# spygaurad/Transformer-CNN-Hybrid-Network-for-Video-Processing

Hardware: AMD Instinct MI355X
Metric: clips/sec fwd+bwd, [B=8,T=16,3,224,224] d=512, 1/2/4/8 MI355X (higher is better)
Workload: dtype bf16; 1 GPU; config 2: clips [8,16,3,224,224] per GPU, CNN 32-64-128-256 + 2-layer transformer d=512 h=8 hid=2048, 8 classes; global_batch=8, frames=16, step=zero_grad+fwd+cross_entropy+bwd+grad_allreduce+adamw, launch=1 replayed hipGraph per step (graph.GraphedTrainStep), optimizer=HybridAdamW (hyb_adamw_step, one launch), parallelism=dp1, train_mode=BatchNorm batch stats, attention dropout 0.1 (reference semantics)

## Files before the change

transformer_cnn_hybrid_network_for_video_processing_amd/csrc/conv_v2.hip:

```cpp
#include <stdlib.h>
#include <type_traits>
#include "hyb_common.h"

namespace {

typedef __attribute__((address_space(3))) void lds_void_t;

template <int N> __device__ __forceinline__ void wait_vmcnt() { asm volatile("s_waitcnt vmcnt(%0)" ::"n"(N) : "memory"); }

__device__ __forceinline__ void dma16(__amdgpu_buffer_rsrc_t rsrc, unsigned voff, unsigned soff, bf16* lds_dst_wave_base) {
    __builtin_amdgcn_raw_ptr_buffer_load_lds(rsrc, (lds_void_t*)lds_dst_wave_base, 16, voff, soff, 0, 0);
}
constexpr unsigned V2_OOB = 0xfffffff0u;
constexpr unsigned V2_RECORDS = 0x80000000u;

template <int S> using step_c = std::integral_constant<int, S>;

template <int NT, int CB, int PGR, int PGC, int R>
struct V2Geom {
    static constexpr int PG = PGR * PGC, MT = 7;
    static constexpr int NW = CB * PG;
    static constexpr int TH = 4 * PGR, TW = 28 * PGC, HH = TH + 2, HW_ = TW + 2, HP = HH * HW_;
    static constexpr int NHW = (HP * 4 + 63) / 64;
    static constexpr int HT = (NHW + NW - 1) / NW;
    static constexpr int HBUF = NHW * 512;
    static constexpr int CBW = CB * NT * 16;
    static constexpr int WSLOT = CBW * 32;
    static constexpr int NWW = CBW / 16;
    static constexpr int WI = NWW >= NW ? NWW / NW : 1;
    static constexpr int NHS = 10 - R;
    static constexpr int STAT_FLOATS = NW * 2 * NT * 16;
    static constexpr size_t LDS_BYTES = (size_t)(2 * HBUF + R * WSLOT) * 2 + STAT_FLOATS * 4;
    static_assert(NW == 8 || NW == 4, "four or eight waves");
    static_assert(LDS_BYTES <= (NW == 8 ? 160 : 80) * 1024, "160 KiB of LDS per CU");
    static_assert(HW_ % 4 == 2, "halo swizzle assumes halo width = 2 mod 4");
    static_assert(R >= 3 && R <= 6, "ring depth");
    static constexpr int hi(int s) { s = ((s % 9) + 9) % 9; return s < NHS ? (HT + NHS - 1 - s) / NHS : 0; }
    static constexpr int hstart(int s) { int a = 0; for (int j = 0; j < s; ++j) a += hi(j); return a; }
    static constexpr int wait_n(int s) {
        int n = hi(s - R + 3);
        for (int j = s - R + 4; j <= s; ++j) n += WI + hi(j);
        return n;
    }
};

template <int NT, int CB, int PGR, int PGC, int R, bool STATS>
__global__ __launch_bounds__(CB * PGR * PGC * 64, CB * PGR * PGC == 4 ? 2 : 1) void conv3x3_v2_kernel(const bf16* __restrict__ x, const bf16* __restrict__ wp,
                                                            bf16* __restrict__ y, float* __restrict__ stats,
                                                            int N, int H, int W, int Cip, int Cop,
                                                            int tilesX, int tilesY, int numTiles, int stat_rows, int xpix, long long xblk) {
    using G = V2Geom<NT, CB, PGR, PGC, R>;
    constexpr int MT = G::MT, TH = G::TH, TW = G::TW, HW_ = G::HW_, HP = G::HP, HT = G::HT, NHW = G::NHW;
    constexpr int CBW = G::CBW, WSLOT = G::WSLOT, NWW = G::NWW, WI = G::WI, PG = G::PG, NW = G::NW, NTHR = NW * 64;
    extern __shared__ __attribute__((aligned(16))) unsigned char smem_raw[];
    bf16* const hbuf = reinterpret_cast<bf16*>(smem_raw);
    bf16* const wring = hbuf + 2 * G::HBUF;
    float* const wgstat = reinterpret_cast<float*>(wring + R * WSLOT);

    const int tid = threadIdx.x;
    const int lane = tid & 63;
    const int wave = __builtin_amdgcn_readfirstlane(tid >> 6);
    const int cb = wave % CB, pg = wave / CB;
    const int prow = pg / PGC, pstrip = pg % PGC;
    const int p = lane & 15, q = lane >> 4, py = p >> 2, px = p & 3;
    const int co_wg = blockIdx.y * CBW;
    const int co_base = co_wg + cb * (NT * 16);
    const int nCblk = Cip / 32;
    const long long wrow = (long long)9 * Cip;

    if (STATS) {
        for (int i = tid; i < G::STAT_FLOATS; i += NTHR) wgstat[i] = 0.f;
    }

    constexpr bool HOFF_REG = true;
    unsigned hoff[HOFF_REG ? HT : 1];
    int hyx[HT];
#pragma unroll
    for (int k = 0; k < HT; ++k) {
        int wi = k * NW + wave;
        if (wi > NHW - 1) wi = NHW - 1;
        const int u = wi * 64 + lane, hp = u >> 2, sp = u & 3;
        const int hy = hp / HW_, hx = hp - hy * HW_;
        const int s = sp ^ ((hy & 1) << 1);
        if (HOFF_REG) hoff[k] = (unsigned)(((hy * W + hx) * xpix + s * 8) * 2);
        hyx[k] = hp < HP ? ((hy << 20) | (hx << 4) | s) : (0x7ff << 20);
    }
    unsigned woff[WI];
    int wdst[WI];
#pragma unroll
    for (int i = 0; i < WI; ++i) {
        const int wi = (i * NW + wave) % NWW;
        const int u = wi * 64 + lane, row = u >> 2, sp = u & 3;
        const int f = (4 - ((row >> 3) & 3)) & 3;
        woff[i] = (unsigned)(((long long)row * wrow + ((sp ^ f) << 3)) * 2);
        wdst[i] = wi * 512;
    }
    const __amdgpu_buffer_rsrc_t wrsrc = hyb_rsrc((wp + (long long)co_wg * wrow), V2_RECORDS);
    const int aoff0 = (cb * (NT * 16) + (p >> 2) * 8 + (p & 3)) * 32 + ((q ^ ((4 - (p >> 2)) & 3)) << 3);
    auto aoff = [&](int t) { return aoff0 + ((t >> 1) * 32 + (t & 1) * 4) * 32; };
    const int lane_el = ((prow * 4 + py) * HW_ + pstrip * 28 + px) * 32;

    struct Blk { int n, ty0, tx0, cblk; };
    auto decode = [&](int tile, int cblk) {
        Blk b;
        b.n = tile / (tilesX * tilesY);
        const int trem = tile - b.n * (tilesX * tilesY);
        b.ty0 = (trem / tilesX) * TH;
        b.tx0 = (trem % tilesX) * TW;
        b.cblk = cblk;
        return b;
    };
    auto halo_rsrc = [&](const Blk& b) {
        const long long base = ((long long)(b.n * H + b.ty0 - 1) * W + (b.tx0 - 1)) * xpix + b.cblk * xblk;
        return hyb_rsrc((x + base), V2_RECORDS);
    };
    auto halo_piece = [&](const Blk& b, __amdgpu_buffer_rsrc_t rs, bf16* hb, int k) {
        const int hy = hyx[k] >> 20, hx = (hyx[k] >> 4) & 0xffff;
        const int gy = b.ty0 - 1 + hy, gx = b.tx0 - 1 + hx;
        const bool valid = ((unsigned)gy < (unsigned)H) && ((unsigned)gx < (unsigned)W);
        const unsigned off = HOFF_REG ? hoff[HOFF_REG ? k : 0] : (unsigned)(((hy * W + hx) * xpix + (hyx[k] & 15) * 8) * 2);
        int wi = k * NW + wave;
        if (wi > NHW - 1) wi = NHW - 1;
        dma16(rs, valid ? off : V2_OOB, 0, hb + wi * 512);
    };
    auto weight_pieces = [&](int cblk, int tap, int slot) {
        const unsigned so = (unsigned)((cblk * 9 + tap) * 64);
#pragma unroll
        for (int i = 0; i < WI; ++i) dma16(wrsrc, woff[i], so, wring + slot * WSLOT + wdst[i]);
    };
    auto bptr_of = [&](const bf16* hb, int tap) {
        const int kh = tap / 3, kw = tap % 3;
        const int sw = ((py + kh) & 1) << 1;
        return hb + lane_el + (kh * HW_ + kw) * 32 + ((q ^ sw) << 3);
    };

    const int tchunk = (numTiles + (int)gridDim.x - 1) / (int)gridDim.x;
    int tile = blockIdx.x * tchunk;
    const int tile_end = tile + tchunk < numTiles ? tile + tchunk : numTiles;
    Blk cur = decode(tile, 0);
    int hsel = 0, slot_cur = 0;
    bool after_store = false;
    constexpr int NS = MT * ((NT + 1) / 2);

    {
        const __amdgpu_buffer_rsrc_t rs0 = halo_rsrc(cur);
#pragma unroll
        for (int k = 0; k < HT; ++k) halo_piece(cur, rs0, hbuf, k);
    }
#pragma unroll
    for (int s = 0; s < R - 1; ++s) weight_pieces(0, s, s);
    wait_vmcnt<0>();
    __builtin_amdgcn_s_barrier();

    Frag<bf16> a_cur[NT], bfr[MT];
#pragma unroll
    for (int t = 0; t < NT; ++t) frag_load(a_cur[t], wring + aoff(t));
    {
        const bf16* bp = bptr_of(hbuf, 0);
#pragma unroll
        for (int m = 0; m < MT; ++m) frag_load(bfr[m], bp + m * 128);
    }

    f32x4 acc[MT][NT];
#pragma unroll
    for (int m = 0; m < MT; ++m)
#pragma unroll
        for (int t = 0; t < NT; ++t) acc[m][t] = f32x4{0.f, 0.f, 0.f, 0.f};

    while (true) {
        const bool last_cblk = cur.cblk + 1 >= nCblk;
        const int ntile = last_cblk ? (tile + 1 < tile_end ? tile + 1 : tile) : tile;
        const Blk nxt = decode(ntile, last_cblk ? 0 : cur.cblk + 1);
        bf16* const hb_cur = hbuf + hsel * G::HBUF;
        bf16* const hb_nxt = hbuf + (hsel ^ 1) * G::HBUF;
        const __amdgpu_buffer_rsrc_t nrs = halo_rsrc(nxt);

        auto step = [&](auto S_) __attribute__((always_inline)) {
            constexpr int S = decltype(S_)::value;
            {
                constexpr int FT = (S + R - 1) % 9;
                const int fc = (S + R - 1 >= 9) ? nxt.cblk : cur.cblk;
                int slot_fill = slot_cur - 1;
                if (slot_fill < 0) slot_fill += R;
                weight_pieces(fc, FT, slot_fill);
#pragma unroll
                for (int k = 0; k < G::hi(S); ++k) halo_piece(nxt, nrs, hb_nxt, G::hstart(S) + k);
            }
            int slot_next = slot_cur + 1;
            if (slot_next >= R) slot_next -= R;
            Frag<bf16> a_nxt[NT];
            {
                const bf16* as = wring + slot_next * WSLOT;
#pragma unroll
                for (int t = 0; t < NT; ++t) frag_load(a_nxt[t], as + aoff(t));
            }
            const bf16* bp = bptr_of(S == 8 ? hb_nxt : hb_cur, (S + 1) % 9);
#pragma unroll
            for (int m = 0; m < MT; ++m) {
#pragma unroll
                for (int t = 0; t < NT; ++t) acc[m][t] = mma32(a_cur[t], bfr[m], acc[m][t]);
                frag_load(bfr[m], bp + m * 128);
            }
#pragma unroll
            for (int m = 0; m < MT; ++m) {
                __builtin_amdgcn_sched_group_barrier(0x008, NT, 0);
                if (m < NT) __builtin_amdgcn_sched_group_barrier(0x100, 2, 0);
                else __builtin_amdgcn_sched_group_barrier(0x100, 1, 0);
            }
#pragma unroll
            for (int t = 0; t < NT; ++t) a_cur[t] = a_nxt[t];
            slot_cur = slot_next;
            if constexpr (S < R - 3) {
                if (after_store) wait_vmcnt<G::wait_n(S) + NS>(); else wait_vmcnt<G::wait_n(S)>();
            } else {
                wait_vmcnt<G::wait_n(S)>();
            }
            __builtin_amdgcn_s_barrier();
        };
        step(step_c<0>{}); step(step_c<1>{}); step(step_c<2>{}); step(step_c<3>{}); step(step_c<4>{});
        step(step_c<5>{}); step(step_c<6>{}); step(step_c<7>{}); step(step_c<8>{});

        if (last_cblk) {
            const int n = cur.n, ty0 = cur.ty0, tx0 = cur.tx0;
            const bool full = (ty0 + TH <= H) && (tx0 + TW <= W);
            float s1[NT][4], s2[NT][4];
            if (STATS) {
#pragma unroll
                for (int t = 0; t < NT; ++t)
#pragma unroll
                    for (int r = 0; r < 4; ++r) { s1[t][r] = 0.f; s2[t][r] = 0.f; }
            }
            const int gy = ty0 + prow * 4 + py;
            auto emit = [&](auto FULL_) __attribute__((always_inline)) {
                constexpr bool FULL = decltype(FULL_)::value;
#pragma unroll
                for (int m = 0; m < MT; ++m) {
                    const int gx = tx0 + pstrip * 28 + m * 4 + px;
                    const bool valid = FULL || ((gy < H) && (gx < W));
                    if (valid) {
                        bf16* dst = y + ((long long)(n * H + gy) * W + gx) * Cop + co_base + q * 8;
#pragma unroll
                        for (int h = 0; h < (NT + 1) / 2; ++h) {
                            Vec8<bf16> v;
#pragma unroll
                            for (int j = 0; j < 8; ++j) v.set(j, acc[m][NT == 1 ? 0 : h * 2 + (j >> 2)][j & 3]);
                            v.store(dst + h * 32);
                        }
                        if (STATS) {
#pragma unroll
                            for (int t = 0; t < NT; ++t)
#pragma unroll
                                for (int r = 0; r < 4; ++r) {
                                    const float v = acc[m][t][r];
                                    s1[t][r] += v;
                                    s2[t][r] = fmaf(v, v, s2[t][r]);
                                }
                        }
                    }
#pragma unroll
                    for (int t = 0; t < NT; ++t) acc[m][t] = f32x4{0.f, 0.f, 0.f, 0.f};
                }
            };
            if (full) {
                emit(std::true_type{});
                after_store = true;
            } else {
                emit(std::false_type{});
                wait_vmcnt<0>();
                after_store = false;
            }
            if (STATS) {
#pragma unroll
                for (int t = 0; t < NT; ++t)
#pragma unroll
                    for (int r = 0; r < 4; ++r) {
                        const float a = row16_sum(s1[t][r]), b = row16_sum(s2[t][r]);
                        if (p == 0) {
                            const int cl = (t >> 1) * 32 + q * 8 + (t & 1) * 4 + r;
                            wgstat[(wave * 2 + 0) * (NT * 16) + cl] += a;
                            wgstat[(wave * 2 + 1) * (NT * 16) + cl] += b;
                        }
                    }
            }
            if (tile + 1 >= tile_end) break;
            ++tile;
        }
        else after_store = false;
        cur = nxt;
        hsel ^= 1;
    }

    wait_vmcnt<0>();
    if (STATS) {
        __syncthreads();
        for (int i = tid; i < 2 * CBW; i += NTHR) {
            const int which = i / CBW, cl = i % CBW;
            const int cbi = cl / (NT * 16), c16 = cl % (NT * 16);
            float a = 0.f;
#pragma unroll
            for (int g = 0; g < PG; ++g) a += wgstat[((g * CB + cbi) * 2 + which) * (NT * 16) + c16];
            stats[((long long)blockIdx.x * 2 + which) * Cop + co_wg + cl] = a;
            for (int rrow = blockIdx.x + gridDim.x; rrow < stat_rows; rrow += gridDim.x) stats[((long long)rrow * 2 + which) * Cop + co_wg + cl] = 0.f;
        }
    }
}

template <int CB, int PGR, int PGC, bool STATS>
__global__ __launch_bounds__(CB * PGR * PGC * 64, 2) void conv3x3_k32_kernel(const bf16* __restrict__ x, const bf16* __restrict__ wp, bf16* __restrict__ y,
                                                                            float* __restrict__ stats, int N, int H, int W, int Cip, int Cop, int tilesX,
                                                                            int tilesY, int numTiles, int stat_rows, int xpix, long long xblk) {
    constexpr int NT = 2, HBN = 3;
    using G = V2Geom<NT, CB, PGR, PGC, 3>;
    constexpr int MT = G::MT, TH = G::TH, TW = G::TW, HW_ = G::HW_, HP = G::HP, HT = G::HT, NHW = G::NHW, CBW = G::CBW, PG = G::PG, NW = G::NW,
                  NTHR = NW * 64;
    static_assert(NW == 4, "two four-wave workgroups per CU");
    extern __shared__ __attribute__((aligned(16))) unsigned char smem_raw[];
    bf16* const hbuf = reinterpret_cast<bf16*>(smem_raw);
    float* const wgstat = reinterpret_cast<float*>(hbuf + HBN * G::HBUF);
    const int tid = threadIdx.x, lane = tid & 63;
    const int wave = __builtin_amdgcn_readfirstlane(tid >> 6);
    const int cb = wave % CB, pg = wave / CB;
    const int prow = pg / PGC, pstrip = pg % PGC;
    const int p = lane & 15, q = lane >> 4, py = p >> 2, px = p & 3;
    const int co_wg = blockIdx.y * CBW;
    const int co_base = co_wg + cb * (NT * 16);
    const long long wrow = (long long)9 * Cip;
    (void)xblk;

    Frag<bf16> aw[9][NT];
#pragma unroll
    for (int t = 0; t < NT; ++t) {
        const bf16* row = wp + (long long)(co_base + (t >> 1) * 32 + (p >> 2) * 8 + (t & 1) * 4 + (p & 3)) * wrow + 8 * q;
#pragma unroll
        for (int tap = 0; tap < 9; ++tap) frag_load(aw[tap][t], row + tap * 32);
    }
    unsigned hoff[HT];
    int hyx[HT];
#pragma unroll
    for (int k = 0; k < HT; ++k) {
        int wi = k * NW + wave;
        if (wi > NHW - 1) wi = NHW - 1;
        const int u = wi * 64 + lane, hp = u >> 2, sp = u & 3;
        const int hy = hp / HW_, hx = hp - hy * HW_;
        const int s = sp ^ ((hy & 1) << 1);
        hoff[k] = (unsigned)(((hy * W + hx) * xpix + s * 8) * 2);
        hyx[k] = hp < HP ? ((hy << 20) | (hx << 4) | s) : (0x7ff << 20);
    }
    const int lane_el = ((prow * 4 + py) * HW_ + pstrip * 28 + px) * 32;
    struct Tl { int n, ty0, tx0; };
    auto decode = [&](int tile) {
        Tl b;
        b.n = tile / (tilesX * tilesY);
        const int trem = tile - b.n * (tilesX * tilesY);
        b.ty0 = (trem / tilesX) * TH;
        b.tx0 = (trem % tilesX) * TW;
        return b;
    };
    auto halo_dma = [&](const Tl& b, bf16* hb) {
        const long long base = ((long long)(b.n * H + b.ty0 - 1) * W + (b.tx0 - 1)) * xpix;
        const __amdgpu_buffer_rsrc_t rs = hyb_rsrc((x + base), V2_RECORDS);
#pragma unroll
        for (int k = 0; k < HT; ++k) {
            const int hy = hyx[k] >> 20, hx = (hyx[k] >> 4) & 0xffff;
            const int gy = b.ty0 - 1 + hy, gx = b.tx0 - 1 + hx;
            const bool valid = ((unsigned)gy < (unsigned)H) && ((unsigned)gx < (unsigned)W);
            int wi = k * NW + wave;
            if (wi > NHW - 1) wi = NHW - 1;
            dma16(rs, valid ? hoff[k] : V2_OOB, 0, hb + wi * 512);
        }
    };
    auto bptr_of = [&](const bf16* hb, int tap) {
        const int kh = tap / 3, kw = tap % 3;
        const int sw = ((py + kh) & 1) << 1;
        return hb + lane_el + (kh * HW_ + kw) * 32 + ((q ^ sw) << 3);
    };

    const int tchunk = (numTiles + (int)gridDim.x - 1) / (int)gridDim.x;
    const int tile0 = blockIdx.x * tchunk;
    const int tile_end = tile0 + tchunk < numTiles ? tile0 + tchunk : numTiles;
    const int ntiles = tile_end - tile0;
    auto tl = [&](int i) { return decode(tile0 + (i < ntiles ? i : ntiles - 1)); };
    constexpr int NS = MT * ((NT + 1) / 2);

    halo_dma(tl(0), hbuf);
    halo_dma(tl(1), hbuf + G::HBUF);
    wait_vmcnt<0>();
    __builtin_amdgcn_s_barrier();

    Frag<bf16> bfr[MT];
    {
        const bf16* bp = bptr_of(hbuf, 0);
#pragma unroll
        for (int m = 0; m < MT; ++m) frag_load(bfr[m], bp + m * 128);
    }
    f32x4 acc[MT][NT];
#pragma unroll
    for (int m = 0; m < MT; ++m)
#pragma unroll
        for (int t = 0; t < NT; ++t) acc[m][t] = f32x4{0.f, 0.f, 0.f, 0.f};
    float s1[NT][4], s2[NT][4];
#pragma unroll
    for (int t = 0; t < NT; ++t)
#pragma unroll
        for (int r = 0; r < 4; ++r) { s1[t][r] = 0.f; s2[t][r] = 0.f; }

    int hsel = 0;
    bool prev_full = false;
    for (int it = 0; it < ntiles; ++it) {
        const Tl cur = tl(it);
        const int h1 = hsel + 1 >= HBN ? 0 : hsel + 1, h2 = h1 + 1 >= HBN ? 0 : h1 + 1;
        const bf16* hb_cur = hbuf + hsel * G::HBUF;
        const bf16* hb_nxt = hbuf + h1 * G::HBUF;
        halo_dma(tl(it + 2), hbuf + h2 * G::HBUF);
#pragma unroll
        for (int tap = 0; tap < 9; ++tap) {
            const bf16* bp = bptr_of(tap == 8 ? hb_nxt : hb_cur, (tap + 1) % 9);
#pragma unroll
            for (int m = 0; m < MT; ++m) {
#pragma unroll
                for (int t = 0; t < NT; ++t) acc[m][t] = mma32(aw[tap][t], bfr[m], acc[m][t]);
                frag_load(bfr[m], bp + m * 128);
            }
#pragma unroll
            for (int m = 0; m < MT; ++m) {
                __builtin_amdgcn_sched_group_barrier(0x008, NT, 0);
                __builtin_amdgcn_sched_group_barrier(0x100, 1, 0);
            }
        }
        const int n = cur.n, ty0 = cur.ty0, tx0 = cur.tx0;
        const bool full = (ty0 + TH <= H) && (tx0 + TW <= W);
        const int gy = ty0 + prow * 4 + py;
        auto emit = [&](auto FULL_) __attribute__((always_inline)) {
            constexpr bool FULL = decltype(FULL_)::value;
#pragma unroll
            for (int m = 0; m < MT; ++m) {
                const int gx = tx0 + pstrip * 28 + m * 4 + px;
                const bool valid = FULL || ((gy < H) && (gx < W));
                if (valid) {
                    bf16* dst = y + ((long long)(n * H + gy) * W + gx) * Cop + co_base + q * 8;
                    Vec8<bf16> v;
#pragma unroll
                    for (int j = 0; j < 8; ++j) v.set(j, acc[m][j >> 2][j & 3]);
                    v.store(dst);
                    if (STATS) {
#pragma unroll
                        for (int t = 0; t < NT; ++t)
#pragma unroll
                            for (int r = 0; r < 4; ++r) {
                                const float a = acc[m][t][r];
                                s1[t][r] += a;
                                s2[t][r] = fmaf(a, a, s2[t][r]);
                            }
                    }
                }
#pragma unroll
                for (int t = 0; t < NT; ++t) acc[m][t] = f32x4{0.f, 0.f, 0.f, 0.f};
            }
        };
        if (full) {
            emit(std::true_type{});
            if (prev_full) wait_vmcnt<HT + 2 * NS>(); else wait_vmcnt<HT + NS>();
        } else {
            emit(std::false_type{});
            wait_vmcnt<0>();
        }
        prev_full = full;
        __builtin_amdgcn_s_barrier();
        hsel = h1;
    }
    wait_vmcnt<0>();
    if (STATS) {
#pragma unroll
        for (int t = 0; t < NT; ++t)
#pragma unroll
            for (int r = 0; r < 4; ++r) {
                const float a = row16_sum(s1[t][r]), b = row16_sum(s2[t][r]);
                if (p == 0) {
                    const int cl = (t >> 1) * 32 + q * 8 + (t & 1) * 4 + r;
                    wgstat[(wave * 2 + 0) * (NT * 16) + cl] = a;
                    wgstat[(wave * 2 + 1) * (NT * 16) + cl] = b;
                }
            }
        __syncthreads();
        for (int i = tid; i < 2 * CBW; i += NTHR) {
            const int which = i / CBW, cl = i % CBW;
            const int cbi = cl / (NT * 16), c16 = cl % (NT * 16);
            float a = 0.f;
#pragma unroll
            for (int g = 0; g < PG; ++g) a += wgstat[((g * CB + cbi) * 2 + which) * (NT * 16) + c16];
            stats[((long long)blockIdx.x * 2 + which) * Cop + co_wg + cl] = a;
            for (int rrow = blockIdx.x + gridDim.x; rrow < stat_rows; rrow += gridDim.x) stats[((long long)rrow * 2 + which) * Cop + co_wg + cl] = 0.f;
        }
    }
}

template <int CB, int PGR, int PGC>
int launch_k32(const bf16* x, const bf16* wp, bf16* y, float* part, int N, int H, int W, int Cip, int Cop, int stat_rows, hipStream_t st, int xpix,
               long long xblk) {
    using G = V2Geom<2, CB, PGR, PGC, 3>;
    constexpr size_t LDS = (size_t)3 * G::HBUF * 2 + G::STAT_FLOATS * 4;
    static_assert(LDS <= 80 * 1024, "two workgroups per CU");
    const int tilesX = hyb_cdiv(W, G::TW), tilesY = hyb_cdiv(H, G::TH);
    const long long numTiles = (long long)N * tilesX * tilesY;
    int gx = (int)(numTiles < 512 ? numTiles : 512);
    if (part && gx > stat_rows) gx = stat_rows;
    if (gx < 1) gx = 1;
    gx = hyb_cdiv(numTiles, hyb_cdiv(numTiles, gx));
    const dim3 grid(gx, Cop / G::CBW);
    static HybAttrOnce once_stats, once_plain;
    if (int e = hyb_set_lds_attr(once_stats, (const void*)conv3x3_k32_kernel<CB, PGR, PGC, true>, (int)LDS)) return e;
    if (int e = hyb_set_lds_attr(once_plain, (const void*)conv3x3_k32_kernel<CB, PGR, PGC, false>, (int)LDS)) return e;
    if (part)
        hipLaunchKernelGGL((conv3x3_k32_kernel<CB, PGR, PGC, true>), grid, dim3(256), LDS, st, x, wp, y, part, N, H, W, Cip, Cop, tilesX, tilesY, (int)numTiles,
                           stat_rows, xpix, xblk);
    else
        hipLaunchKernelGGL((conv3x3_k32_kernel<CB, PGR, PGC, false>), grid, dim3(256), LDS, st, x, wp, y, (float*)nullptr, N, H, W, Cip, Cop, tilesX, tilesY,
                           (int)numTiles, 0, xpix, xblk);
    HYB_LAUNCH_CHECK();
    return 0;
}

template <int NT, int CB, int PGR, int PGC, int R>
int launch_v2(const bf16* x, const bf16* wp, bf16* y, float* part, int N, int H, int W, int Cip, int Cop, int stat_rows, hipStream_t st, int xpix,
              long long xblk) {
    using G = V2Geom<NT, CB, PGR, PGC, R>;
    const int tilesX = hyb_cdiv(W, G::TW), tilesY = hyb_cdiv(H, G::TH);
    const long long numTiles = (long long)N * tilesX * tilesY;
    constexpr int SLOTS = G::NW == 8 ? 256 : 512;
    int gx = (int)(numTiles < SLOTS ? numTiles : SLOTS);
    if (part && gx > stat_rows) gx = stat_rows;
    if (gx < 1) gx = 1;
    gx = hyb_cdiv(numTiles, hyb_cdiv(numTiles, gx));
    const dim3 grid(gx, Cop / G::CBW);
    static HybAttrOnce once_stats, once_plain;
    if (int e = hyb_set_lds_attr(once_stats, (const void*)conv3x3_v2_kernel<NT, CB, PGR, PGC, R, true>, (int)G::LDS_BYTES)) return e;
    if (int e = hyb_set_lds_attr(once_plain, (const void*)conv3x3_v2_kernel<NT, CB, PGR, PGC, R, false>, (int)G::LDS_BYTES)) return e;
    if (part)
        hipLaunchKernelGGL((conv3x3_v2_kernel<NT, CB, PGR, PGC, R, true>), grid, dim3(G::NW * 64), G::LDS_BYTES, st, x, wp, y, part, N, H, W, Cip, Cop,
                           tilesX, tilesY, (int)numTiles, stat_rows, xpix, xblk);
    else
        hipLaunchKernelGGL((conv3x3_v2_kernel<NT, CB, PGR, PGC, R, false>), grid, dim3(G::NW * 64), G::LDS_BYTES, st, x, wp, y, (float*)nullptr, N, H, W,
                           Cip, Cop, tilesX, tilesY, (int)numTiles, 0, xpix, xblk);
    HYB_LAUNCH_CHECK();
    return 0;
}

double v2_cost(int N, int H, int W, int TH, int TW, int gy) {
    const long long tiles = (long long)N * hyb_cdiv(W, TW) * hyb_cdiv(H, TH) * gy;
    const long long rounds = (tiles + 255) / 256;
    return (double)rounds * TH * TW;
}

}

int hyb_conv_v2_supported(int W, int Cip, int Cop) {
    return !(Cip % 32 != 0 || (long long)40 * W * Cip >= (1ll << 29) || (long long)256 * 9 * Cip >= (1ll << 29)) && Cop % 32 == 0;
}

int hyb_conv_v2(const void* x, const void* wp, void* y, float* part, int N, int H, int W, int Cip, int Cop, int stat_rows, hipStream_t st, long long xblk) {
    const int xpix = xblk ? 32 : Cip;
    if (!xblk) xblk = 32;
    if (Cip % 32 != 0 || (long long)40 * W * Cip >= (1ll << 29) || (long long)256 * 9 * Cip >= (1ll << 29)) return -100;
    const bf16* xb = (const bf16*)x; const bf16* wb = (const bf16*)wp; bf16* yb = (bf16*)y;
#define V2(NT_, CB_, PGR_, PGC_, R_) launch_v2<NT_, CB_, PGR_, PGC_, R_>(xb, wb, yb, part, N, H, W, Cip, Cop, stat_rows, st, xpix, xblk)
    static const int nw_env = getenv("HYB_V2_NW") ? atoi(getenv("HYB_V2_NW")) : 0;
    const int nw = nw_env ? nw_env : (Cop % 256 == 0 ? 8 : 4);
    static const int k32_env = getenv("HYB_CONV_K32") ? atoi(getenv("HYB_CONV_K32")) : 1;
    if (k32_env && nw == 4 && Cip == 32 && Cop % 64 == 0) {
        return v2_cost(N, H, W, 8, 28, Cop / 64) <= v2_cost(N, H, W, 4, 56, Cop / 64)
                   ? launch_k32<2, 2, 1>(xb, wb, yb, part, N, H, W, Cip, Cop, stat_rows, st, xpix, xblk)
                   : launch_k32<2, 1, 2>(xb, wb, yb, part, N, H, W, Cip, Cop, stat_rows, st, xpix, xblk);
    }
    if (nw == 4) {
        if (Cop % 256 == 0) return V2(4, 4, 1, 1, 3);
        if (Cop % 128 == 0) return v2_cost(N, H, W, 8, 28, Cop / 128) <= v2_cost(N, H, W, 4, 56, Cop / 128) ? V2(4, 2, 2, 1, 4) : V2(4, 2, 1, 2, 4);
        if (Cop % 64 == 0) return v2_cost(N, H, W, 8, 28, Cop / 64) <= v2_cost(N, H, W, 4, 56, Cop / 64) ? V2(2, 2, 2, 1, 4) : V2(2, 2, 1, 2, 4);
        if (Cop % 32 == 0) return V2(2, 1, 4, 1, 4);
        return -100;
    }
    if (Cop % 256 == 0) {
        return v2_cost(N, H, W, 8, 28, Cop / 256) <= v2_cost(N, H, W, 4, 56, Cop / 256) ? V2(4, 4, 2, 1, 6) : V2(4, 4, 1, 2, 6);
    }
    if (Cop % 128 == 0) {
        return v2_cost(N, H, W, 16, 28, Cop / 128) <= v2_cost(N, H, W, 8, 56, Cop / 128) ? V2(4, 2, 4, 1, 6) : V2(4, 2, 2, 2, 6);
    }
    if (Cop % 64 == 0) return V2(4, 1, 4, 2, 5);
    if (Cop % 32 == 0) return V2(2, 1, 4, 2, 6);
#undef V2
    return -100;
}
```

Baseline: 6085 clips/s.

## Add 8-wave single-workgroup conv3x3 v3 kernel with row-streamed weight ring

Adds a conv3x3 kernel that runs one 512-thread workgroup per CU over four pixel groups. Weights are streamed one kernel row at a time through a three-slot LDS ring, and input halos are double-buffered, so DMA for the next row or channel block overlaps the MFMA work of the current one. The dispatcher sends Cop==128, Cip>=256 convolutions (such as the 256->128 data-gradient conv) to this kernel when 16-row tiles cost less than 8-row tiles. It trades the two-workgroups-per-CU occupancy of v2 for larger tiles with more weight reuse, which risks weaker latency hiding.

```diff
diff --git a/transformer_cnn_hybrid_network_for_video_processing_amd/csrc/conv_v2.hip b/transformer_cnn_hybrid_network_for_video_processing_amd/csrc/conv_v2.hip
--- a/transformer_cnn_hybrid_network_for_video_processing_amd/csrc/conv_v2.hip
+++ b/transformer_cnn_hybrid_network_for_video_processing_amd/csrc/conv_v2.hip
@@ -305,6 +305,285 @@
     }
 }
 
+template <int NT, int CB, int PGR, int PGC>
+struct V3Geom : V2Geom<NT, CB, PGR, PGC, 3> {
+    using B = V2Geom<NT, CB, PGR, PGC, 3>;
+    static constexpr int R = 3;
+    static constexpr int RSLOT = 3 * B::WSLOT;
+    static constexpr int WPS = 3 * B::WI;
+    static constexpr size_t LDS_BYTES = (size_t)(2 * B::HBUF + R * RSLOT) * 2 + B::STAT_FLOATS * 4;
+    static_assert(B::NW == 8 && B::PG == 4, "one 8-wave workgroup per CU, four pixel groups");
+    static_assert(LDS_BYTES <= 160 * 1024, "160 KiB of LDS per CU");
+    static_assert(B::HH <= 18, "32-bit halo offsets: hyb_conv_v2_supported bounds 40 * W * Cip");
+    static constexpr int wait_n(int s) { return (s == 0 ? B::HT : 0) + WPS; }
+    static_assert(wait_n(0) + B::MT * ((NT + 1) / 2) <= 63, "vmcnt range");
+};
+
+template <int NT, int CB, int PGR, int PGC, bool STATS>
+__global__ __launch_bounds__(512, 1) void conv3x3_v3_kernel(const bf16* __restrict__ x, const bf16* __restrict__ wp, bf16* __restrict__ y,
+                                                            float* __restrict__ stats, int N, int H, int W, int Cip, int Cop, int tilesX, int tilesY,
+                                                            int numTiles, int stat_rows, int xpix, long long xblk) {
+    using G = V3Geom<NT, CB, PGR, PGC>;
+    constexpr int MT = G::MT, TH = G::TH, TW = G::TW, HW_ = G::HW_, HP = G::HP, HT = G::HT, NHW = G::NHW;
+    constexpr int CBW = G::CBW, WSLOT = G::WSLOT, RSLOT = G::RSLOT, NWW = G::NWW, WI = G::WI, PG = G::PG, NW = G::NW, R = G::R, NTHR = NW * 64;
+    extern __shared__ __attribute__((aligned(16))) unsigned char smem_raw[];
+    bf16* const hbuf = reinterpret_cast<bf16*>(smem_raw);
+    bf16* const wring = hbuf + 2 * G::HBUF;
+    float* const wgstat = reinterpret_cast<float*>(wring + R * RSLOT);
+
+    const int tid = threadIdx.x;
+    const int lane = tid & 63;
+    const int wave = __builtin_amdgcn_readfirstlane(tid >> 6);
+    const int cb = wave % CB, pg = wave / CB;
+    const int prow = pg / PGC, pstrip = pg % PGC;
+    const int p = lane & 15, q = lane >> 4, py = p >> 2, px = p & 3;
+    const int co_wg = blockIdx.y * CBW;
+    const int co_base = co_wg + cb * (NT * 16);
+    const int nCblk = Cip / 32;
+    const long long wrow = (long long)9 * Cip;
+
+    if (STATS) {
+        for (int i = tid; i < G::STAT_FLOATS; i += NTHR) wgstat[i] = 0.f;
+    }
+
+    unsigned hoff[HT];
+    int hyx[HT];
+#pragma unroll
+    for (int k = 0; k < HT; ++k) {
+        int wi = k * NW + wave;
+        if (wi > NHW - 1) wi = NHW - 1;
+        const int u = wi * 64 + lane, hp = u >> 2, sp = u & 3;
+        const int hy = hp / HW_, hx = hp - hy * HW_;
+        const int s = sp ^ ((hy & 1) << 1);
+        hoff[k] = (unsigned)(((hy * W + hx) * xpix + s * 8) * 2);
+        hyx[k] = hp < HP ? ((hy << 20) | (hx << 4) | s) : (0x7ff << 20);
+    }
+    unsigned woff[WI];
+    int wdst[WI];
+#pragma unroll
+    for (int i = 0; i < WI; ++i) {
+        const int wi = (i * NW + wave) % NWW;
+        const int u = wi * 64 + lane, row = u >> 2, sp = u & 3;
+        const int f = (4 - ((row >> 3) & 3)) & 3;
+        woff[i] = (unsigned)(((long long)row * wrow + ((sp ^ f) << 3)) * 2);
+        wdst[i] = wi * 512;
+    }
+    const __amdgpu_buffer_rsrc_t wrsrc = hyb_rsrc((wp + (long long)co_wg * wrow), V2_RECORDS);
+    const int aoff0 = (cb * (NT * 16) + (p >> 2) * 8 + (p & 3)) * 32 + ((q ^ ((4 - (p >> 2)) & 3)) << 3);
+    auto aoff = [&](int t) { return aoff0 + ((t >> 1) * 32 + (t & 1) * 4) * 32; };
+    const int lane_el = ((prow * 4 + py) * HW_ + pstrip * 28 + px) * 32;
+
+    struct Blk { int n, ty0, tx0, cblk; };
+    auto decode = [&](int tile, int cblk) {
+        Blk b;
+        b.n = tile / (tilesX * tilesY);
+        const int trem = tile - b.n * (tilesX * tilesY);
+        b.ty0 = (trem / tilesX) * TH;
+        b.tx0 = (trem % tilesX) * TW;
+        b.cblk = cblk;
+        return b;
+    };
+    auto halo_dma = [&](const Blk& b, bf16* hb) {
+        const long long base = ((long long)(b.n * H + b.ty0 - 1) * W + (b.tx0 - 1)) * xpix + b.cblk * xblk;
+        const __amdgpu_buffer_rsrc_t rs = hyb_rsrc((x + base), V2_RECORDS);
+#pragma unroll
+        for (int k = 0; k < HT; ++k) {
+            const int hy = hyx[k] >> 20, hx = (hyx[k] >> 4) & 0xffff;
+            const int gy = b.ty0 - 1 + hy, gx = b.tx0 - 1 + hx;
+            const bool valid = ((unsigned)gy < (unsigned)H) && ((unsigned)gx < (unsigned)W);
+            int wi = k * NW + wave;
+            if (wi > NHW - 1) wi = NHW - 1;
+            dma16(rs, valid ? hoff[k] : V2_OOB, 0, hb + wi * 512);
+        }
+    };
+    auto weight_row = [&](int cblk, int kh, int slot) {
+#pragma unroll
+        for (int kw = 0; kw < 3; ++kw) {
+            const unsigned so = (unsigned)((cblk * 9 + kh * 3 + kw) * 64);
+#pragma unroll
+            for (int i = 0; i < WI; ++i) dma16(wrsrc, woff[i], so, wring + slot * RSLOT + kw * WSLOT + wdst[i]);
+        }
+    };
+    auto bptr_of = [&](const bf16* hb, int tap) {
+        const int kh = tap / 3, kw = tap % 3;
+        const int sw = ((py + kh) & 1) << 1;
+        return hb + lane_el + (kh * HW_ + kw) * 32 + ((q ^ sw) << 3);
+    };
+
+    const int tchunk = (numTiles + (int)gridDim.x - 1) / (int)gridDim.x;
+    int tile = blockIdx.x * tchunk;
+    const int tile_end = tile + tchunk < numTiles ? tile + tchunk : numTiles;
+    Blk cur = decode(tile, 0);
+    int hsel = 0, slot_cur = 0;
+    bool after_store = false;
+    constexpr int NS = MT * ((NT + 1) / 2);
+
+    halo_dma(cur, hbuf);
+    weight_row(0, 0, 0);
+    weight_row(0, 1, 1);
+    wait_vmcnt<0>();
+    __builtin_amdgcn_s_barrier();
+
+    Frag<bf16> bfr[MT];
+    {
+        const bf16* bp = bptr_of(hbuf, 0);
+#pragma unroll
+        for (int m = 0; m < MT; ++m) frag_load(bfr[m], bp + m * 128);
+    }
+    f32x4 acc[MT][NT];
+#pragma unroll
+    for (int m = 0; m < MT; ++m)
+#pragma unroll
+        for (int t = 0; t < NT; ++t) acc[m][t] = f32x4{0.f, 0.f, 0.f, 0.f};
+
+    while (true) {
+        const bool last_cblk = cur.cblk + 1 >= nCblk;
+        const int ntile = last_cblk ? (tile + 1 < tile_end ? tile + 1 : tile) : tile;
+        const Blk nxt = decode(ntile, last_cblk ? 0 : cur.cblk + 1);
+        bf16* const hb_cur = hbuf + hsel * G::HBUF;
+        bf16* const hb_nxt = hbuf + (hsel ^ 1) * G::HBUF;
+        const bool active = cur.ty0 + prow * 4 < H;
+
+        auto step = [&](auto S_) __attribute__((always_inline)) {
+            constexpr int S = decltype(S_)::value;
+            const bf16* const ws = wring + slot_cur * RSLOT;
+            Frag<bf16> a_cur[NT], a_nxt[NT];
+            if (active) {
+#pragma unroll
+                for (int t = 0; t < NT; ++t) frag_load(a_cur[t], ws + aoff(t));
+            }
+            if constexpr (S == 0) halo_dma(nxt, hb_nxt);
+            {
+                int slot_fill = slot_cur - 1;
+                if (slot_fill < 0) slot_fill += R;
+                weight_row(S == 0 ? cur.cblk : nxt.cblk, (S + 2) % 3, slot_fill);
+            }
+            if (active) {
+#pragma unroll
+                for (int kw = 0; kw < 3; ++kw) {
+                    if (kw < 2) {
+#pragma unroll
+                        for (int t = 0; t < NT; ++t) frag_load(a_nxt[t], ws + (kw + 1) * WSLOT + aoff(t));
+                    }
+                    const int tap = S * 3 + kw;
+                    const bf16* bp = bptr_of(tap == 8 ? hb_nxt : hb_cur, (tap + 1) % 9);
+#pragma unroll
+                    for (int m = 0; m < MT; ++m) {
+#pragma unroll
+                        for (int t = 0; t < NT; ++t) acc[m][t] = mma32(a_cur[t], bfr[m], acc[m][t]);
+                        frag_load(bfr[m], bp + m * 128);
+                    }
+#pragma unroll
+                    for (int m = 0; m < MT; ++m) {
+                        __builtin_amdgcn_sched_group_barrier(0x008, NT, 0);
+                        if (kw < 2 && m < NT) __builtin_amdgcn_sched_group_barrier(0x100, 2, 0);
+                        else __builtin_amdgcn_sched_group_barrier(0x100, 1, 0);
+                    }
+                    if (kw < 2) {
+#pragma unroll
+                        for (int t = 0; t < NT; ++t) a_cur[t] = a_nxt[t];
+                    }
+                }
+            } else if constexpr (S == 2) {
+                const bf16* bp = bptr_of(hb_nxt, 0);
+#pragma unroll
+                for (int m = 0; m < MT; ++m) frag_load(bfr[m], bp + m * 128);
+            }
+            slot_cur = slot_cur + 1 >= R ? 0 : slot_cur + 1;
+            if constexpr (S == 0) {
+                if (after_store) wait_vmcnt<G::wait_n(0) + NS>(); else wait_vmcnt<G::wait_n(0)>();
+            } else {
+                wait_vmcnt<G::wait_n(S)>();
+            }
+            __builtin_amdgcn_s_barrier();
+        };
+        step(step_c<0>{}); step(step_c<1>{}); step(step_c<2>{});
+
+        if (last_cblk) {
+            const int n = cur.n, ty0 = cur.ty0, tx0 = cur.tx0;
+            const bool full = (ty0 + TH <= H) && (tx0 + TW <= W);
+            float s1[NT][4], s2[NT][4];
+            if (STATS) {
+#pragma unroll
+                for (int t = 0; t < NT; ++t)
+#pragma unroll
+                    for (int r = 0; r < 4; ++r) { s1[t][r] = 0.f; s2[t][r] = 0.f; }
+            }
+            const int gy = ty0 + prow * 4 + py;
+            auto emit = [&](auto FULL_) __attribute__((always_inline)) {
+                constexpr bool FULL = decltype(FULL_)::value;
+#pragma unroll
+                for (int m = 0; m < MT; ++m) {
+                    const int gx = tx0 + pstrip * 28 + m * 4 + px;
+                    const bool valid = FULL || ((gy < H) && (gx < W));
+                    if (valid) {
+                        bf16* dst = y + ((long long)(n * H + gy) * W + gx) * Cop + co_base + q * 8;
+#pragma unroll
+                        for (int h = 0; h < (NT + 1) / 2; ++h) {
+                            Vec8<bf16> v;
+#pragma unroll
+                            for (int j = 0; j < 8; ++j) v.set(j, acc[m][NT == 1 ? 0 : h * 2 + (j >> 2)][j & 3]);
+                            v.store(dst + h * 32);
+                        }
+                        if (STATS) {
+#pragma unroll
+                            for (int t = 0; t < NT; ++t)
+#pragma unroll
+                                for (int r = 0; r < 4; ++r) {
+                                    const float v = acc[m][t][r];
+                                    s1[t][r] += v;
+                                    s2[t][r] = fmaf(v, v, s2[t][r]);
+                                }
+                        }
+                    }
+#pragma unroll
+                    for (int t = 0; t < NT; ++t) acc[m][t] = f32x4{0.f, 0.f, 0.f, 0.f};
+                }
+            };
+            if (full) {
+                emit(std::true_type{});
+                after_store = true;
+            } else {
+                emit(std::false_type{});
+                wait_vmcnt<0>();
+                after_store = false;
+            }
+            if (STATS) {
+#pragma unroll
+                for (int t = 0; t < NT; ++t)
+#pragma unroll
+                    for (int r = 0; r < 4; ++r) {
+                        const float a = row16_sum(s1[t][r]), b = row16_sum(s2[t][r]);
+                        if (p == 0) {
+                            const int cl = (t >> 1) * 32 + q * 8 + (t & 1) * 4 + r;
+                            wgstat[(wave * 2 + 0) * (NT * 16) + cl] += a;
+                            wgstat[(wave * 2 + 1) * (NT * 16) + cl] += b;
+                        }
+                    }
+            }
+            if (tile + 1 >= tile_end) break;
+            ++tile;
+        }
+        else after_store = false;
+        cur = nxt;
+        hsel ^= 1;
+    }
+
+    wait_vmcnt<0>();
+    if (STATS) {
+        __syncthreads();
+        for (int i = tid; i < 2 * CBW; i += NTHR) {
+            const int which = i / CBW, cl = i % CBW;
+            const int cbi = cl / (NT * 16), c16 = cl % (NT * 16);
+            float a = 0.f;
+#pragma unroll
+            for (int g = 0; g < PG; ++g) a += wgstat[((g * CB + cbi) * 2 + which) * (NT * 16) + c16];
+            stats[((long long)blockIdx.x * 2 + which) * Cop + co_wg + cl] = a;
+            for (int rrow = blockIdx.x + gridDim.x; rrow < stat_rows; rrow += gridDim.x) stats[((long long)rrow * 2 + which) * Cop + co_wg + cl] = 0.f;
+        }
+    }
+}
+
 template <int CB, int PGR, int PGC, bool STATS>
 __global__ __launch_bounds__(CB * PGR * PGC * 64, 2) void conv3x3_k32_kernel(const bf16* __restrict__ x, const bf16* __restrict__ wp, bf16* __restrict__ y,
                                                                             float* __restrict__ stats, int N, int H, int W, int Cip, int Cop, int tilesX,
@@ -545,6 +824,30 @@
     return 0;
 }
 
+template <int NT, int CB, int PGR, int PGC>
+int launch_v3(const bf16* x, const bf16* wp, bf16* y, float* part, int N, int H, int W, int Cip, int Cop, int stat_rows, hipStream_t st, int xpix,
+              long long xblk) {
+    using G = V3Geom<NT, CB, PGR, PGC>;
+    const int tilesX = hyb_cdiv(W, G::TW), tilesY = hyb_cdiv(H, G::TH);
+    const long long numTiles = (long long)N * tilesX * tilesY;
+    int gx = (int)(numTiles < 256 ? numTiles : 256);
+    if (part && gx > stat_rows) gx = stat_rows;
+    if (gx < 1) gx = 1;
+    gx = hyb_cdiv(numTiles, hyb_cdiv(numTiles, gx));
+    const dim3 grid(gx, Cop / G::CBW);
+    static HybAttrOnce once_stats, once_plain;
+    if (int e = hyb_set_lds_attr(once_stats, (const void*)conv3x3_v3_kernel<NT, CB, PGR, PGC, true>, (int)G::LDS_BYTES)) return e;
+    if (int e = hyb_set_lds_attr(once_plain, (const void*)conv3x3_v3_kernel<NT, CB, PGR, PGC, false>, (int)G::LDS_BYTES)) return e;
+    if (part)
+        hipLaunchKernelGGL((conv3x3_v3_kernel<NT, CB, PGR, PGC, true>), grid, dim3(512), G::LDS_BYTES, st, x, wp, y, part, N, H, W, Cip, Cop, tilesX,
+                           tilesY, (int)numTiles, stat_rows, xpix, xblk);
+    else
+        hipLaunchKernelGGL((conv3x3_v3_kernel<NT, CB, PGR, PGC, false>), grid, dim3(512), G::LDS_BYTES, st, x, wp, y, (float*)nullptr, N, H, W, Cip,
+                           Cop, tilesX, tilesY, (int)numTiles, 0, xpix, xblk);
+    HYB_LAUNCH_CHECK();
+    return 0;
+}
+
 double v2_cost(int N, int H, int W, int TH, int TW, int gy) {
     const long long tiles = (long long)N * hyb_cdiv(W, TW) * hyb_cdiv(H, TH) * gy;
     const long long rounds = (tiles + 255) / 256;
@@ -563,6 +866,15 @@
     if (Cip % 32 != 0 || (long long)40 * W * Cip >= (1ll << 29) || (long long)256 * 9 * Cip >= (1ll << 29)) return -100;
     const bf16* xb = (const bf16*)x; const bf16* wb = (const bf16*)wp; bf16* yb = (bf16*)y;
 #define V2(NT_, CB_, PGR_, PGC_, R_) launch_v2<NT_, CB_, PGR_, PGC_, R_>(xb, wb, yb, part, N, H, W, Cip, Cop, stat_rows, st, xpix, xblk)
+    static const int v3_env = getenv("HYB_CONV_V3") ? atoi(getenv("HYB_CONV_V3")) : 1;
+    const double c16 = v2_cost(N, H, W, 16, 28, 1), c8 = v2_cost(N, H, W, 8, 56, 1);
+    const bool rows16 = c16 <= c8;
+    if (v3_env && Cip >= 64 && Cop % 64 == 0 && (v3_env == 2 || (Cop == 128 && Cip >= 256 && c16 < c8))) {
+        if (Cop % 128 == 0) return rows16 ? launch_v3<4, 2, 4, 1>(xb, wb, yb, part, N, H, W, Cip, Cop, stat_rows, st, xpix, xblk)
+                                          : launch_v3<4, 2, 2, 2>(xb, wb, yb, part, N, H, W, Cip, Cop, stat_rows, st, xpix, xblk);
+        return rows16 ? launch_v3<2, 2, 4, 1>(xb, wb, yb, part, N, H, W, Cip, Cop, stat_rows, st, xpix, xblk)
+                      : launch_v3<2, 2, 2, 2>(xb, wb, yb, part, N, H, W, Cip, Cop, stat_rows, st, xpix, xblk);
+    }
     static const int nw_env = getenv("HYB_V2_NW") ? atoi(getenv("HYB_V2_NW")) : 0;
     const int nw = nw_env ? nw_env : (Cop % 256 == 0 ? 8 : 4);
     static const int k32_env = getenv("HYB_CONV_K32") ? atoi(getenv("HYB_CONV_K32")) : 1;
```

Result: no change. 6090 clips/s, median of 3 (+0.1%).
